# razvanmatisan/duodiff

Hardware: AMD Instinct MI355X
Metric: images/sec (whole node) DuoDiff 1000-step CelebA-64 (higher is better)
Workload: dtype bf16

## Files before the change

duodiff_amd/csrc/attention.hip:

```cpp
#include "dd_internal.h"

#include <type_traits>
#include <utility>

namespace dd {
namespace {

constexpr int kMaxKeyTiles = 9;
constexpr int kLP = kMaxKeyTiles * 32;
constexpr int kHD = 64;
constexpr int kPartBytes = 4 * 2 * 66 * 4;

__device__ __forceinline__ unsigned pack2_bf16(float lo, float hi) {
    typedef __bf16 bf16v2 __attribute__((ext_vector_type(2)));
    typedef float f32v2 __attribute__((ext_vector_type(2)));
    const f32v2 q = {lo, hi};
    return __builtin_bit_cast(unsigned, __builtin_convertvector(q, bf16v2));
}

__device__ __forceinline__ unsigned lds_addr_of(const void* p) {
    return (unsigned)(size_t)(const __attribute__((address_space(3))) char*)p;
}

__device__ __forceinline__ int k_swz(int r) { return ((r >> 1) & 7) ^ ((r & 1) << 2); }
__device__ __forceinline__ int v_swz(int r) { return (2 * (r & 3)) ^ ((r >> 2) & 1); }

template <typename T> struct AttnLayout;
template <> struct AttnLayout<bf16_t> {
    static constexpr int kRowK = 128;
    static constexpr int kRowV = 128;
    static constexpr int kVBytes = kLP * kRowV;
};
template <> struct AttnLayout<float> {
    static constexpr int kRowK = 256 + 16;
    static constexpr int kRowV = kLP * 4 + 16;
    static constexpr int kVBytes = kHD * kRowV;
};

template <typename T, int NKT, int NT, bool KPERM, typename TileFn>
__device__ __forceinline__ void attend_tiles(const char* Ks, const char* Vt, int L, int nkt, int lane, TileFn&& tile,
                                         const f32x4 (&qcur)[sizeof(T) == 2 ? 4 : 8], f32x16 (&o)[2], float& mx, float& sum) {
    using Lay = AttnLayout<T>;
    const int half = lane >> 5, r32 = lane & 31;
    const f32x16 zero16 = {0.f, 0.f, 0.f, 0.f, 0.f, 0.f, 0.f, 0.f, 0.f, 0.f, 0.f, 0.f, 0.f, 0.f, 0.f, 0.f};
    f32x16 s[NT];

    if constexpr (sizeof(T) == 2) {
        bf16x8 qf[4];
#pragma unroll
        for (int st = 0; st < 4; ++st) qf[st] = __builtin_bit_cast(bf16x8, qcur[st]);
        auto load_k = [&](int t, bf16x8 (&kf)[4]) {
            const char* kr = Ks + (t * 32 + r32) * Lay::kRowK;
            const int sw = k_swz(r32);
#pragma unroll
            for (int st = 0; st < 4; ++st) {
                const int ch = KPERM ? 4 * (st >> 1) + 2 * half + (st & 1) : 2 * st + half;
                kf[st] = *reinterpret_cast<const bf16x8*>(kr + ((ch ^ sw) << 4));
            }
        };
        bf16x8 kfa[4], kfb[4];
        if (tile(0) >= 0) load_k(tile(0), kfa);
#pragma unroll
        for (int k = 0; k < NT; ++k) {
            const int t = tile(k);
            const int tn = k + 1 < NT ? tile(k + 1) : -1;
            if (tn >= 0) { if (k & 1) load_k(tn, kfa); else load_k(tn, kfb); }
            __builtin_amdgcn_sched_barrier(0);
            if (t >= 0) {
                s[k] = __builtin_amdgcn_mfma_f32_32x32x16_bf16((k & 1) ? kfb[0] : kfa[0], qf[0], zero16, 0, 0, 0);
#pragma unroll
                for (int st = 1; st < 4; ++st)
                    s[k] = __builtin_amdgcn_mfma_f32_32x32x16_bf16((k & 1) ? kfb[st] : kfa[st], qf[st], s[k], 0, 0, 0);
            } else {
                s[k] = zero16;
            }
            __builtin_amdgcn_sched_barrier(0);
        }
    } else {
#pragma unroll
        for (int k = 0; k < NT; ++k) {
            const int t = tile(k);
            s[k] = zero16;
            if (t >= 0) {
                const char* kr = Ks + (t * 32 + r32) * Lay::kRowK + (32 * half) * 4;
#pragma unroll
                for (int g = 0; g < 8; ++g) {
                    const f32x4 kf = *reinterpret_cast<const f32x4*>(kr + g * 16);
#pragma unroll
                    for (int e = 0; e < 4; ++e)
                        s[k] = __builtin_amdgcn_mfma_f32_32x32x2f32(kf[e], qcur[g][e], s[k], 0, 0, 0);
                }
            }
        }
    }

    mx = -INFINITY;
#pragma unroll
    for (int k = 0; k < NT; ++k) {
        const int t = tile(k);
        if (t >= 0) {
            if (t == nkt - 1) {
#pragma unroll
                for (int e = 0; e < 16; ++e) {
                    const int key = t * 32 + (e & 3) + 8 * (e >> 2) + 4 * half;
                    if (key >= L) s[k][e] = -INFINITY;
                }
            }
#pragma unroll
            for (int e = 0; e < 16; ++e) mx = fmaxf(mx, s[k][e]);
        }
    }
    mx = fmaxf(mx, __shfl_xor(mx, 32));
    constexpr float kScaleLog2e = 0.125f * 1.4426950408889634f;
    const float mxs = mx * kScaleLog2e;
    sum = 0.f;
#pragma unroll
    for (int k = 0; k < NT; ++k) {
        if (tile(k) >= 0) {
#pragma unroll
            for (int e = 0; e < 16; ++e) {
                float p;
                if (NKT == 9 && NT == 9 && k == 8 && e >= 2) {
                    s[k][e] = 0.f;
                    continue;
                }
                if constexpr (sizeof(T) == 2) p = __builtin_amdgcn_exp2f(fmaf(s[k][e], kScaleLog2e, -mxs));
                else p = expf((s[k][e] - mx) * 0.125f);
                s[k][e] = p;
                sum += p;
            }
        }
    }
    sum += __shfl_xor(sum, 32);

    o[0] = zero16;
    o[1] = zero16;

    if constexpr (sizeof(T) == 2) {
        typedef __attribute__((ext_vector_type(4))) short s4;
        struct VF { s4 lo[2][2], hi[2][2]; };
        const int tq = (lane >> 2) & 3, tp = lane & 3, dhalf = (lane >> 4) & 1;
        const char* vb0 = Vt + (4 * half + tq) * Lay::kRowV + 8 * (tp & 1);
        const int vsw = v_swz(4 * half + tq);
        const char* vbd[2] = {vb0 + (((2 * dhalf + (tp >> 1)) ^ vsw) << 4), vb0 + (((4 + 2 * dhalf + (tp >> 1)) ^ vsw) << 4)};
        typedef __attribute__((address_space(3))) s4* lds_s4_ptr;
        auto load_v = [&](int t, VF& f) {
#pragma unroll
            for (int st = 0; st < 2; ++st)
#pragma unroll
                for (int dt = 0; dt < 2; ++dt) {
                    const char* vr = vbd[dt] + (t * 32 + 16 * st) * Lay::kRowV;
                    f.lo[st][dt] = __builtin_amdgcn_ds_read_tr16_b64_v4i16((lds_s4_ptr)(size_t)lds_addr_of(vr));
                    f.hi[st][dt] = __builtin_amdgcn_ds_read_tr16_b64_v4i16((lds_s4_ptr)(size_t)lds_addr_of(vr + 8 * Lay::kRowV));
                }
        };
        VF va, vb;
        if (tile(0) >= 0) load_v(tile(0), va);
#pragma unroll
        for (int k = 0; k < NT; ++k) {
            const int t = tile(k);
            const int tn = k + 1 < NT ? tile(k + 1) : -1;
            if (tn >= 0) { if (k & 1) load_v(tn, va); else load_v(tn, vb); }
            __builtin_amdgcn_sched_barrier(0);
            if (t >= 0) {
                const VF& f = (k & 1) ? vb : va;
#pragma unroll
                for (int st = 0; st < 2; ++st) {
                    bf16x8 pf;
#pragma unroll
                    for (int j = 0; j < 8; ++j) pf[j] = (short)f2bf(s[k][8 * st + j]);
#pragma unroll
                    for (int dt = 0; dt < 2; ++dt) {
                        bf16x8 vf;
#pragma unroll
                        for (int j = 0; j < 4; ++j) { vf[j] = f.lo[st][dt][j]; vf[4 + j] = f.hi[st][dt][j]; }
                        o[dt] = __builtin_amdgcn_mfma_f32_32x32x16_bf16(vf, pf, o[dt], 0, 0, 0);
                    }
                }
            }
            __builtin_amdgcn_sched_barrier(0);
        }
    } else {
#pragma unroll
        for (int k = 0; k < NT; ++k) {
            const int t = tile(k);
            if (t >= 0) {
#pragma unroll
                for (int g = 0; g < 4; ++g) {
#pragma unroll
                    for (int dt = 0; dt < 2; ++dt) {
                        const char* vr = Vt + (dt * 32 + r32) * Lay::kRowV + (t * 32 + 8 * g + 4 * half) * 4;
                        const f32x4 vf = *reinterpret_cast<const f32x4*>(vr);
#pragma unroll
                        for (int e = 0; e < 4; ++e)
                            o[dt] = __builtin_amdgcn_mfma_f32_32x32x2f32(vf[e], s[k][4 * g + e], o[dt], 0, 0, 0);
                    }
                }
            }
        }
    }
}

template <typename T, int NKT>
__global__ void __launch_bounds__(256, sizeof(T) == 2 ? 2 : 1)
attention_kernel(const T* __restrict__ qkv, T* __restrict__ out, int B, int L, int H, int D, int Lp) {
    using Lay = AttnLayout<T>;
    extern __shared__ __attribute__((aligned(16))) char smem[];
    char* Ks = smem;
    char* Vt = smem + kLP * Lay::kRowK;

    const int b = blockIdx.x / H, hh = blockIdx.x % H;
    const int tid = threadIdx.x, lane = tid & 63, wave = tid >> 6;
    const int half = lane >> 5, r32 = lane & 31;
    constexpr long long ld = kHD;
    const long long unit = (long long)Lp * kHD;
    const T* qbase = qkv + ((long long)b * 3 * H + hh) * unit;
    const T* kbase = qbase + (long long)H * unit;
    const T* vbase = kbase + (long long)H * unit;
    const int nkt = NKT > 0 ? NKT : (L + 31) / 32;
    constexpr int EPC = 16 / (int)sizeof(T);
    constexpr int CPR = kHD / EPC;

    constexpr int NQF = sizeof(T) == 2 ? 4 : 8;
    auto load_q = [&](int qc, f32x4 (&qf)[NQF]) {
        const int q = qc * 32 + r32;
        const T* qrow = qbase + (long long)(q < L ? q : L - 1) * ld;
#pragma unroll
        for (int i = 0; i < NQF; ++i)
            qf[i] = sizeof(T) == 2 ? *reinterpret_cast<const f32x4*>(qrow + 16 * i + 8 * half)
                                   : *reinterpret_cast<const f32x4*>(qrow + 32 * half + 4 * i);
    };
    f32x4 qnext[NQF];
    load_q(wave, qnext);

    if constexpr (sizeof(T) == 2) {
        typedef const __attribute__((address_space(1))) void* gptr_t;
        typedef __attribute__((address_space(3))) void* lptr_t;
        const int np = Lp >> 3;
        const int wv = __builtin_amdgcn_readfirstlane(wave);
        const int lr = lane >> 3, slot = lane & 7;
        constexpr int MAXP = (kLP / 8 * 2 + 3) / 4;
#pragma unroll
        for (int i = 0; i < MAXP; ++i) {
            const int p2 = wv + 4 * i;
            if (p2 < 2 * np) {
                const bool isv = p2 >= np;
                const int p = isv ? p2 - np : p2, r = 8 * p + lr;
                const int ch = isv ? (slot ^ v_swz(r)) : (slot ^ k_swz(r));
                const T* src = (isv ? vbase : kbase) + (long long)(r < L ? r : L - 1) * kHD + ch * 8;
                char* dst = (isv ? Vt : Ks) + p * 1024;
                __builtin_amdgcn_global_load_lds((gptr_t)src, (lptr_t)dst, 16, 0, 0);
            }
        }
        for (int i = tid; i < (nkt * 32 - Lp) * 16; i += 256) {
            const int rr = Lp + (i >> 4), c = i & 15;
            *reinterpret_cast<f32x4*>((c < 8 ? Ks : Vt) + rr * 128 + (c & 7) * 16) = f32x4{0.f, 0.f, 0.f, 0.f};
        }
        asm volatile("s_waitcnt vmcnt(0)" ::: "memory");
    } else {
        for (int idx = tid; idx < nkt * 32 * CPR; idx += 256) {
            const int key = idx / CPR, ch = idx % CPR;
            f32x4 kv = {0.f, 0.f, 0.f, 0.f}, vv = {0.f, 0.f, 0.f, 0.f};
            if (key < L) {
                kv = *reinterpret_cast<const f32x4*>(kbase + (long long)key * ld + ch * EPC);
                vv = *reinterpret_cast<const f32x4*>(vbase + (long long)key * ld + ch * EPC);
            }
            *reinterpret_cast<f32x4*>(Ks + key * Lay::kRowK + ch * 16) = kv;
            T tmp[EPC];
            *reinterpret_cast<f32x4*>(tmp) = vv;
#pragma unroll
            for (int e = 0; e < EPC; ++e)
                *reinterpret_cast<T*>(Vt + (ch * EPC + e) * Lay::kRowV + key * (int)sizeof(T)) = tmp[e];
        }
    }

    __syncthreads();

    constexpr bool SPLIT_LAST = NKT == 9;
    const int nqc = (L + 31) / 32;
    const int n_regular = SPLIT_LAST ? 8 : nqc;
    for (int qc = wave; qc < n_regular; qc += 4) {
        const int q = qc * 32 + r32;
        f32x4 qcur[NQF];
#pragma unroll
        for (int i = 0; i < NQF; ++i) qcur[i] = qnext[i];
        if (qc + 4 < n_regular) load_q(qc + 4, qnext);
        else if (SPLIT_LAST) load_q(8, qnext);

        f32x16 o[2];
        float mx, sum;
        attend_tiles<T, NKT, kMaxKeyTiles, false>(Ks, Vt, L, nkt, lane, [&](int k) { return k < nkt ? k : -1; }, qcur, o, mx, sum);
        const float inv = 1.0f / sum;

        T* orow = out + ((long long)b * L + (q < L ? q : L - 1)) * D + hh * kHD;
        if constexpr (sizeof(T) == 2) {
#pragma unroll
            for (int dt = 0; dt < 2; ++dt) {
                uint2 v[4];
#pragma unroll
                for (int g = 0; g < 4; ++g) {
                    bf16_t v4[4];
#pragma unroll
                    for (int e = 0; e < 4; ++e) v4[e] = f2bf(o[dt][4 * g + e] * inv);
                    v[g] = *reinterpret_cast<const uint2*>(v4);
                }
#pragma unroll
                for (int gp = 0; gp < 4; gp += 2) {
                    const auto s0 = __builtin_amdgcn_permlane32_swap(v[gp].x, v[gp + 1].x, false, false);
                    const auto s1 = __builtin_amdgcn_permlane32_swap(v[gp].y, v[gp + 1].y, false, false);
                    const uint4 o4 = {s0[0], s1[0], s0[1], s1[1]};
                    if (q < L) *reinterpret_cast<uint4*>(orow + dt * 32 + 8 * gp + 8 * half) = o4;
                }
            }
        } else if (q < L) {
#pragma unroll
            for (int dt = 0; dt < 2; ++dt)
#pragma unroll
                for (int g = 0; g < 4; ++g) {
                    const int d = dt * 32 + 8 * g + 4 * half;
                    *reinterpret_cast<f32x4*>(orow + d) = f32x4{o[dt][4 * g] * inv, o[dt][4 * g + 1] * inv, o[dt][4 * g + 2] * inv, o[dt][4 * g + 3] * inv};
                }
        }
    }

    if constexpr (SPLIT_LAST) {
        float* part = reinterpret_cast<float*>(smem + kLP * Lay::kRowK + Lay::kVBytes);
        const int rem = L - 256;
        f32x16 o[2];
        float mx, sum;
        attend_tiles<T, NKT, 3, false>(Ks, Vt, L, nkt, lane, [&](int k) { return k < 2 ? wave + 4 * k : (wave == 3 ? 8 : -1); }, qnext, o, mx, sum);
        if (r32 < rem) {
            float* pw = part + (wave * 2 + r32) * 66;
#pragma unroll
            for (int dt = 0; dt < 2; ++dt)
#pragma unroll
                for (int g = 0; g < 4; ++g)
                    *reinterpret_cast<f32x4*>(pw + dt * 32 + 8 * g + 4 * half) =
                        f32x4{o[dt][4 * g], o[dt][4 * g + 1], o[dt][4 * g + 2], o[dt][4 * g + 3]};
            if (half == 0) { pw[64] = mx; pw[65] = sum; }
        }
        __syncthreads();
        if (tid < rem * 64) {
            const int qi = tid >> 6, d = tid & 63;
            float m[4], M = -INFINITY;
#pragma unroll
            for (int w = 0; w < 4; ++w) { m[w] = part[(w * 2 + qi) * 66 + 64]; M = fmaxf(M, m[w]); }
            float num = 0.f, den = 0.f;
#pragma unroll
            for (int w = 0; w < 4; ++w) {
                float f;
                if constexpr (sizeof(T) == 2) f = __builtin_amdgcn_exp2f((m[w] - M) * (0.125f * 1.4426950408889634f));
                else f = expf((m[w] - M) * 0.125f);
                num = fmaf(f, part[(w * 2 + qi) * 66 + d], num);
                den = fmaf(f, part[(w * 2 + qi) * 66 + 65], den);
            }
            out[((long long)b * L + 256 + qi) * D + hh * kHD + d] = Elem<T>::from_f32(num / den);
        }
    }
}


struct QkvAttnArgs {
    const bf16_t* h;
    const bf16_t* wimg;
    const float* bias;
    const bf16_t* hx;
    const float* xres;
    const float* ln_g;
    const float* ln_b;
    bf16_t* out;
    int B, L, H, Lp, E;
};

constexpr int kQaPxBytes = 8 * 6 * 2 * 32 * 4;
constexpr int kQaHxPad = 64;
constexpr int kQaHxBytes = 2 * (1024 * 2 + kQaHxPad);
constexpr int kQaAuxBytes = kQaPxBytes + kQaHxBytes + 256;
constexpr int kQaKQ = 8;
constexpr int kQaBlk = 2 * kQaKQ * 1024;
constexpr int kQaRing = 4 * kQaBlk;
static_assert(8 * 2 * 66 * 4 <= kQaPxBytes, "the split chunk's partials reuse the px area");

typedef const __attribute__((address_space(1))) void* qa_gptr_t;
typedef __attribute__((address_space(3))) void* qa_lptr_t;

constexpr int qa_dma_ops(int b, int nb) { return b < nb ? 2 : 0; }
constexpr int qa_pref_ops(int b, int nb) { return (b >= 0 && b % 3 == 0 && b / 3 + 1 < nb / 3) ? kQaKQ : 0; }
constexpr int qa_younger_dma(int b, int nb) { return qa_pref_ops(b - 1, nb) + qa_dma_ops(b + 2, nb) + qa_pref_ops(b, nb); }
constexpr int qa_younger_rows(int b, int nb) { return qa_dma_ops(b, nb) + qa_dma_ops(b + 1, nb) + qa_dma_ops(b + 2, nb); }

template <int D>
__global__ void __launch_bounds__(512, 1) qkv_attention_kernel(const QkvAttnArgs a) {
    using Lay = AttnLayout<bf16_t>;
    constexpr int KS = D / 16, NS = KS / kQaKQ, NB = 3 * NS;
    static_assert(D % 128 == 0 && D >= 512 && D <= 1024, "k range in slices of 8 k-steps; hxl holds two rows of D <= 1024");
    extern __shared__ __attribute__((aligned(16))) char smem[];
    char* Ks = smem;
    char* Vt = smem + kLP * Lay::kRowK;
    float* px = reinterpret_cast<float*>(smem + kLP * Lay::kRowK + Lay::kVBytes);
    float* part = px;
    char* hxl = smem + kLP * Lay::kRowK + Lay::kVBytes + kQaPxBytes;
    char* qxl = hxl + kQaHxBytes;
    char* ring = smem + kLP * Lay::kRowK + Lay::kVBytes + kQaAuxBytes;

    int b, hh;
    if ((a.B & 7) == 0) { const int slot = blockIdx.x >> 3; b = (blockIdx.x & 7) + 8 * (slot / a.H); hh = slot % a.H; }
    else { b = blockIdx.x / a.H; hh = blockIdx.x % a.H; }
    const int tid = threadIdx.x, lane = tid & 63, wave = __builtin_amdgcn_readfirstlane(tid >> 6);
    const int half = lane >> 5, r32 = lane & 31;
    const int L = a.L, E = a.E;

    const char* wsrc = reinterpret_cast<const char*>(a.wimg) + (size_t)hh * NB * kQaBlk;
    const unsigned lane16 = lane * 16;
    auto dma_block = [&](int bb) {
#pragma unroll
        for (int i = 0; i < 2; ++i) {
            const int pc = wave * 2 + i;
            const char* sb = wsrc + (size_t)bb * kQaBlk + pc * 1024;
            const unsigned lds = lds_addr_of(ring + (bb & 3) * kQaBlk + pc * 1024);
            asm volatile("s_mov_b32 m0, %0\n\tglobal_load_lds_dwordx4 %1, %2" ::"s"(lds), "v"(lane16), "s"(sb) : "memory", "m0");
        }
    };
    dma_block(0);
    dma_block(1);
    dma_block(2);

    const int row = 32 * wave + r32;
    const bf16x8* hfr_u = reinterpret_cast<const bf16x8*>(a.h) + ((long long)b * 8 + wave) * KS * 64;
    const bf16x8* hfr = hfr_u + lane;
    bf16x8 xs[2][kQaKQ];
#pragma unroll
    for (int ks = 0; ks < kQaKQ; ++ks) xs[0][ks] = hfr[ks * 64];

    if (a.hx) {
        for (int i = tid; i < E * (D / 8); i += 512) {
            const int e = i / (D / 8), cch = i % (D / 8);
            *reinterpret_cast<f32x4*>(hxl + e * (D * 2 + kQaHxPad) + cch * 16) = *reinterpret_cast<const f32x4*>(a.hx + ((long long)b * L + e) * D + cch * 8);
        }
    } else if (wave < E) {
        constexpr int NV = D / 256;
        const float* xr = a.xres + ((long long)b * L + wave) * D + lane * (D / 64);
        f32x4 xv[NV];
        float s1 = 0.f;
#pragma unroll
        for (int v = 0; v < NV; ++v) {
            xv[v] = *reinterpret_cast<const f32x4*>(xr + 4 * v);
            s1 += (xv[v][0] + xv[v][1]) + (xv[v][2] + xv[v][3]);
        }
#pragma unroll
        for (int o = 32; o >= 1; o >>= 1) s1 += __shfl_xor(s1, o);
        const float mean = s1 / (float)D;
        float s2 = 0.f;
#pragma unroll
        for (int v = 0; v < NV; ++v) {
            xv[v] = xv[v] - mean;
            s2 += (xv[v][0] * xv[v][0] + xv[v][1] * xv[v][1]) + (xv[v][2] * xv[v][2] + xv[v][3] * xv[v][3]);
        }
#pragma unroll
        for (int o = 32; o >= 1; o >>= 1) s2 += __shfl_xor(s2, o);
        const float rstd = 1.0f / sqrtf(s2 / (float)D + 1e-5f);
#pragma unroll
        for (int v = 0; v < NV; ++v) {
            const f32x4 g = *reinterpret_cast<const f32x4*>(a.ln_g + lane * (D / 64) + 4 * v), c0 = *reinterpret_cast<const f32x4*>(a.ln_b + lane * (D / 64) + 4 * v);
            const f32x4 y = xv[v] * rstd * g + c0;
            *reinterpret_cast<uint2*>(hxl + wave * (D * 2 + kQaHxPad) + (lane * (D / 64) + 4 * v) * 2) = uint2{pack2_bf16(y[0], y[1]), pack2_bf16(y[2], y[3])};
        }
    }
    for (int i = tid; i < (kLP - 256 - E) * 16; i += 512) {
        const int r = 256 + E + (i >> 4), c = i & 15;
        *reinterpret_cast<f32x4*>((c < 8 ? Ks : Vt) + r * 128 + (c & 7) * 16) = f32x4{0.f, 0.f, 0.f, 0.f};
    }

    const f32x16 zero16 = {0.f, 0.f, 0.f, 0.f, 0.f, 0.f, 0.f, 0.f, 0.f, 0.f, 0.f, 0.f, 0.f, 0.f, 0.f, 0.f};
    f32x16 acc[6];
#pragma unroll
    for (int j = 0; j < 6; ++j) acc[j] = zero16;
    f32x4 accx[6];
#pragma unroll
    for (int j = 0; j < 6; ++j) accx[j] = f32x4{0.f, 0.f, 0.f, 0.f};
    const int xg = lane >> 4, xn = lane & 15;
    const int wx16 = (2 * (wave >> 1) + (xg >> 1)) * 1024 + ((16 * (wave & 1) + xn) + 32 * (xg & 1)) * 16;
    const char* hx16 = hxl + (xn < E ? xn : 0) * (D * 2 + kQaHxPad) + (wave >> 1) * 64 + xg * 16;
    bf16x8 wq[4];
    asm volatile("s_waitcnt vmcnt(0)\n\ts_waitcnt lgkmcnt(0)\n\ts_barrier" ::: "memory");
#pragma unroll
    for (int i = 0; i < 4; ++i) wq[i] = *reinterpret_cast<const bf16x8*>(ring + lane * 16 + i * 1024);
    [&]<int... BI>(std::integer_sequence<int, BI...>) {
        ([&] {
            constexpr int bb = BI, q = bb / 3, jj = bb % 3, S = q & 1;
            if constexpr (jj == 0) {
                if constexpr (q > 0) {
                    asm volatile("s_waitcnt vmcnt(%8)"
                                 : "+v"(xs[S][0]), "+v"(xs[S][1]), "+v"(xs[S][2]), "+v"(xs[S][3]), "+v"(xs[S][4]), "+v"(xs[S][5]), "+v"(xs[S][6]), "+v"(xs[S][7])
                                 : "i"(qa_younger_rows(bb, NB)));
                }
                if constexpr (q + 1 < NS) {
#pragma unroll
                    for (int ks = 0; ks < kQaKQ; ++ks)
                        asm volatile("global_load_dwordx4 %0, %1, %2" : "=v"(xs[S ^ 1][ks]) : "v"(lane16), "s"(hfr_u + ((q + 1) * kQaKQ + ks) * 64) : "memory");
                }
            }
            const char* wb = ring + (bb & 3) * kQaBlk + lane * 16;
            const char* wbn = ring + ((bb + 1) & 3) * kQaBlk + lane * 16;
#pragma unroll
            for (int f = 0; f < 2 * kQaKQ; ++f) {
                if (f == kQaKQ) {
                    if constexpr (bb + 1 < NB) {
                        if constexpr (bb + 1 >= 3) asm volatile("s_waitcnt vmcnt(%0)\n\ts_barrier" ::"i"(qa_younger_dma(bb, NB)) : "memory");
                        else asm volatile("s_barrier" ::: "memory");
                    }
                    if constexpr (bb + 3 < NB) dma_block(bb + 3);
                    const bf16x8 hb = *reinterpret_cast<const bf16x8*>(hx16 + q * (kQaKQ * 32));
#pragma unroll
                    for (int t = 0; t < 2; ++t) {
                        const bf16x8 wa = *reinterpret_cast<const bf16x8*>(ring + (bb & 3) * kQaBlk + t * (kQaKQ * 1024) + wx16);
                        accx[2 * jj + t] = __builtin_amdgcn_mfma_f32_16x16x32_bf16(wa, hb, accx[2 * jj + t], 0, 0, 0);
                    }
                }
                const bf16x8 w0 = wq[f & 3];
                if (f + 4 < 2 * kQaKQ) wq[f & 3] = *reinterpret_cast<const bf16x8*>(wb + (f + 4) * 1024);
                else if (bb + 1 < NB) wq[f & 3] = *reinterpret_cast<const bf16x8*>(wbn + (f + 4 - 2 * kQaKQ) * 1024);
                acc[2 * jj + (f >> 3)] = __builtin_amdgcn_mfma_f32_32x32x16_bf16(w0, xs[S][f & 7], acc[2 * jj + (f >> 3)], 0, 0, 0);
            }
        }(), ...);
    }(std::make_integer_sequence<int, NB>{});

    if (xn < E) {
#pragma unroll
        for (int j = 0; j < 6; ++j) *reinterpret_cast<f32x4*>(px + (((wave * 6 + j) * 2 + xn) * 16 + 4 * xg)) = accx[j];
    }
    f32x4 qcur[4];
    const int swk = k_swz(row), swv = v_swz(row);
#pragma unroll
    for (int j = 0; j < 6; ++j) {
        if (a.bias) {
            const float* bj = a.bias + (j >> 1) * D + hh * kHD + 32 * (j & 1) + 4 * half;
#pragma unroll
            for (int g = 0; g < 4; ++g) {
                const f32x4 bv = *reinterpret_cast<const f32x4*>(bj + 8 * g);
#pragma unroll
                for (int e = 0; e < 4; ++e) acc[j][4 * g + e] += bv[e];
            }
        }
        unsigned pk[8];
#pragma unroll
        for (int i = 0; i < 8; ++i) pk[i] = pack2_bf16(acc[j][2 * i], acc[j][2 * i + 1]);
        const int T = j & 1;
        if (j < 2) {
            qcur[2 * T] = __builtin_bit_cast(f32x4, uint4{pk[0], pk[1], pk[2], pk[3]});
            qcur[2 * T + 1] = __builtin_bit_cast(f32x4, uint4{pk[4], pk[5], pk[6], pk[7]});
        } else if (j < 4) {
            *reinterpret_cast<uint4*>(Ks + row * 128 + (((4 * T + 2 * half) ^ swk) << 4)) = uint4{pk[0], pk[1], pk[2], pk[3]};
            *reinterpret_cast<uint4*>(Ks + row * 128 + (((4 * T + 2 * half + 1) ^ swk) << 4)) = uint4{pk[4], pk[5], pk[6], pk[7]};
        } else {
#pragma unroll
            for (int gp = 0; gp < 4; gp += 2) {
                const auto s0 = __builtin_amdgcn_permlane32_swap(pk[2 * gp], pk[2 * gp + 2], false, false);
                const auto s1 = __builtin_amdgcn_permlane32_swap(pk[2 * gp + 1], pk[2 * gp + 3], false, false);
                *reinterpret_cast<uint4*>(Vt + row * 128 + (((4 * T + gp + half) ^ swv) << 4)) = uint4{s0[0], s1[0], s0[1], s1[1]};
            }
        }
    }
    __syncthreads();
    if (tid < E * 192) {
        const int e = tid / 192, c = tid % 192, j = c >> 5, col = c & 31;
        float v = a.bias ? a.bias[(j >> 1) * D + hh * kHD + 32 * (j & 1) + col] : 0.f;
#pragma unroll
        for (int kb = 0; kb < 4; ++kb) v += px[(((2 * kb + (col >> 4)) * 6 + j) * 2 + e) * 16 + (col & 15)];
        const bf16_t vb = f2bf(v);
        const int d = 32 * (j & 1) + col, r = 256 + e;
        if (j < 2) {
            *reinterpret_cast<bf16_t*>(qxl + e * 128 + d * 2) = vb;
        } else if (j < 4) {
            const int T = d >> 5, dd = d & 31, hf = (dd >> 2) & 1, ae = (dd & 3) + 4 * (dd >> 3);
            *reinterpret_cast<bf16_t*>(Ks + r * 128 + (((4 * T + 2 * hf + (ae >> 3)) ^ k_swz(r)) << 4) + (ae & 7) * 2) = vb;
        } else {
            *reinterpret_cast<bf16_t*>(Vt + r * 128 + (((d >> 3) ^ v_swz(r)) << 4) + (d & 7) * 2) = vb;
        }
    }
    __syncthreads();

    f32x4 qe[4];
    {
        const bf16_t* qrow = reinterpret_cast<const bf16_t*>(qxl) + (r32 < E ? r32 : E - 1) * kHD + 4 * half;
#pragma unroll
        for (int st = 0; st < 4; ++st) {
            const uint2 lo = *reinterpret_cast<const uint2*>(qrow + 32 * (st >> 1) + 16 * (st & 1));
            const uint2 hi = *reinterpret_cast<const uint2*>(qrow + 32 * (st >> 1) + 16 * (st & 1) + 8);
            qe[st] = __builtin_bit_cast(f32x4, uint4{lo.x, lo.y, hi.x, hi.y});
        }
    }

    {
        f32x16 o[2];
        float mx, sum;
        attend_tiles<bf16_t, 9, kMaxKeyTiles, true>(Ks, Vt, L, kMaxKeyTiles, lane, [&](int k) { return k; }, qcur, o, mx, sum);
        const float inv = 1.0f / sum;
        bf16_t* orow = a.out + ((long long)b * L + E + row) * D + hh * kHD;
#pragma unroll
        for (int dt = 0; dt < 2; ++dt) {
            uint2 v[4];
#pragma unroll
            for (int g = 0; g < 4; ++g) {
                bf16_t v4[4];
#pragma unroll
                for (int e = 0; e < 4; ++e) v4[e] = f2bf(o[dt][4 * g + e] * inv);
                v[g] = *reinterpret_cast<const uint2*>(v4);
            }
#pragma unroll
            for (int gp = 0; gp < 4; gp += 2) {
                const auto s0 = __builtin_amdgcn_permlane32_swap(v[gp].x, v[gp + 1].x, false, false);
                const auto s1 = __builtin_amdgcn_permlane32_swap(v[gp].y, v[gp + 1].y, false, false);
                *reinterpret_cast<uint4*>(orow + dt * 32 + 8 * gp + 8 * half) = uint4{s0[0], s1[0], s0[1], s1[1]};
            }
        }
    }

    {
        f32x16 o[2];
        float mx, sum;
        attend_tiles<bf16_t, 9, 2, true>(Ks, Vt, L, kMaxKeyTiles, lane, [&](int k) { return k == 0 ? wave : (wave == 7 ? 8 : -1); }, qe, o, mx, sum);
        if (r32 < E) {
            float* pw = part + (wave * 2 + r32) * 66;
#pragma unroll
            for (int dt = 0; dt < 2; ++dt)
#pragma unroll
                for (int g = 0; g < 4; ++g)
                    *reinterpret_cast<f32x4*>(pw + dt * 32 + 8 * g + 4 * half) =
                        f32x4{o[dt][4 * g], o[dt][4 * g + 1], o[dt][4 * g + 2], o[dt][4 * g + 3]};
            if (half == 0) { pw[64] = mx; pw[65] = sum; }
        }
        __syncthreads();
        if (tid < E * 64) {
            const int qi = tid >> 6, d = tid & 63;
            float m[8], M = -INFINITY;
#pragma unroll
            for (int w = 0; w < 8; ++w) { m[w] = part[(w * 2 + qi) * 66 + 64]; M = fmaxf(M, m[w]); }
            float num = 0.f, den = 0.f;
#pragma unroll
            for (int w = 0; w < 8; ++w) {
                const float f = __builtin_amdgcn_exp2f((m[w] - M) * (0.125f * 1.4426950408889634f));
                num = fmaf(f, part[(w * 2 + qi) * 66 + d], num);
                den = fmaf(f, part[(w * 2 + qi) * 66 + 65], den);
            }
            a.out[((long long)b * L + qi) * D + hh * kHD + d] = f2bf(num / den);
        }
    }
}

}

template <typename T>
hipError_t launch_attention(const T* qkv, T* out, int B, int L, int H, int D, hipStream_t s) {
    if (L > kLP || D != H * kHD || L < 1) return hipErrorInvalidValue;
    using Lay = AttnLayout<T>;
    const size_t lds = (size_t)kLP * Lay::kRowK + (size_t)Lay::kVBytes + kPartBytes;
    const int Lp = make_head_major(L, H).Lp;
    if (L == 257 || L == 258) hipLaunchKernelGGL((attention_kernel<T, 9>), dim3(B * H), dim3(256), lds, s, qkv, out, B, L, H, D, Lp);
    else hipLaunchKernelGGL((attention_kernel<T, 0>), dim3(B * H), dim3(256), lds, s, qkv, out, B, L, H, D, Lp);
    return hipGetLastError();
}

void qkv_attention_pack(int D, int H, const float* w, unsigned short (*to_bf16)(float), unsigned short* img) {
    const int NS = D / 16 / kQaKQ;
    for (int hh = 0; hh < H; ++hh)
        for (int q = 0; q < NS; ++q)
            for (int j = 0; j < 6; ++j)
                for (int ks = 0; ks < kQaKQ; ++ks)
                    for (int lane = 0; lane < 64; ++lane) {
                        const float* src = w + ((size_t)(j >> 1) * D + 64 * hh + 32 * (j & 1) + (lane & 31)) * D + 16 * (q * kQaKQ + ks) + 8 * (lane >> 5);
                        unsigned short* dst = img + (((((size_t)hh * NS + q) * 6 + j) * kQaKQ + ks) * 64 + lane) * 8;
                        for (int i = 0; i < 8; ++i) dst[i] = to_bf16(src[i]);
                    }
}

bool qkv_attention_supported(int D, int H, int L, int extras) {
    return (D == 512 || D == 768 || D == 1024) && H * kHD == D && (extras == 1 || extras == 2) && L == 256 + extras;
}

static size_t qkv_attention_lds() { return (size_t)kLP * AttnLayout<bf16_t>::kRowK + AttnLayout<bf16_t>::kVBytes + kQaAuxBytes + kQaRing; }

hipError_t launch_qkv_attention(const bf16_t* h, const bf16_t* wimg, const float* bias, const bf16_t* hx, const float* xres,
                                const float* ln_g, const float* ln_b, bf16_t* out, int B, int L, int H, int D, int extras, hipStream_t s) {
    if (!qkv_attention_supported(D, H, L, extras) || !h || !wimg || (!hx && (!xres || !ln_g || !ln_b)) || !out || B < 1) return hipErrorInvalidValue;
    const QkvAttnArgs a{h, wimg, bias, hx, xres, ln_g, ln_b, out, B, L, H, make_head_major(L, H).Lp, extras};
    switch (D) {
        case 512: hipLaunchKernelGGL((qkv_attention_kernel<512>), dim3(B * H), dim3(512), qkv_attention_lds(), s, a); break;
        case 768: hipLaunchKernelGGL((qkv_attention_kernel<768>), dim3(B * H), dim3(512), qkv_attention_lds(), s, a); break;
        default: hipLaunchKernelGGL((qkv_attention_kernel<1024>), dim3(B * H), dim3(512), qkv_attention_lds(), s, a); break;
    }
    return hipGetLastError();
}

hipError_t init_attention_kernels() {
    for (const void* f : {(const void*)qkv_attention_kernel<512>, (const void*)qkv_attention_kernel<768>, (const void*)qkv_attention_kernel<1024>})
        if (hipError_t e = hipFuncSetAttribute(f, hipFuncAttributeMaxDynamicSharedMemorySize, (int)qkv_attention_lds()); e != hipSuccess) return e;
    const int lb = kLP * AttnLayout<bf16_t>::kRowK + AttnLayout<bf16_t>::kVBytes + kPartBytes;
    const int lf = kLP * AttnLayout<float>::kRowK + AttnLayout<float>::kVBytes + kPartBytes;
    hipError_t e = hipFuncSetAttribute((const void*)attention_kernel<bf16_t, 9>, hipFuncAttributeMaxDynamicSharedMemorySize, lb);
    if (e == hipSuccess) e = hipFuncSetAttribute((const void*)attention_kernel<bf16_t, 0>, hipFuncAttributeMaxDynamicSharedMemorySize, lb);
    if (e == hipSuccess) e = hipFuncSetAttribute((const void*)attention_kernel<float, 9>, hipFuncAttributeMaxDynamicSharedMemorySize, lf);
    if (e == hipSuccess) e = hipFuncSetAttribute((const void*)attention_kernel<float, 0>, hipFuncAttributeMaxDynamicSharedMemorySize, lf);
    return e;
}

template hipError_t launch_attention<bf16_t>(const bf16_t*, bf16_t*, int, int, int, int, hipStream_t);
template hipError_t launch_attention<float>(const float*, float*, int, int, int, int, hipStream_t);

}
```

duodiff_amd/csrc/gemm.hip:

```cpp
#include "dd_internal.h"

#include <type_traits>

namespace dd {

namespace {

typedef const __attribute__((address_space(1))) void* gptr_t;
typedef __attribute__((address_space(3))) void* lptr_t;

__device__ __forceinline__ void glds16(const void* src, void* lds_dst) {
    __builtin_amdgcn_global_load_lds((gptr_t)src, (lptr_t)lds_dst, 16, 0, 0);
}

__device__ __forceinline__ float gelu_erf_f32(float v) { return 0.5f * v * (1.0f + erff(v * 0.70710678118654752440f)); }

__device__ __forceinline__ void glds16s(const char* sbase, unsigned voff, const void* lds_dst) {
    const unsigned lds = (unsigned)(size_t)(const __attribute__((address_space(3))) char*)lds_dst;
    asm volatile("s_mov_b32 m0, %0\n\tglobal_load_lds_dwordx4 %1, %2" ::"s"(lds), "v"(voff), "s"(sbase) : "memory", "m0");
}

template <int ROWS, int NWAVES>
__device__ __forceinline__ void stage_tile(const char* g, long long row_stride, char* lds_tile,
                                           int wave, int lane, int row_limit) {
    constexpr int PER_WAVE = ROWS / 8 / NWAVES;
#pragma unroll
    for (int j = 0; j < PER_WAVE; ++j) {
        const int inst = wave * PER_WAVE + j;
        int r = inst * 8 + (lane >> 3);
        const int c = (lane & 7) ^ ((r >> 1) & 7);
        r = r < row_limit ? r : row_limit - 1;
        glds16(g + (long long)r * row_stride + c * 16, lds_tile + inst * 1024);
    }
}

template <typename T>
__device__ __forceinline__ f32x4 gelu_erf4(f32x4 v) {
    if constexpr (sizeof(T) == 4) {
        f32x4 r;
#pragma unroll
        for (int e = 0; e < 4; ++e) r[e] = gelu_erf_f32(v[e]);
        return r;
    } else {
        f32x4 sc;
#pragma unroll
        for (int i = 0; i < 4; ++i) sc[i] = __builtin_amdgcn_fmed3f(v[i], -3.8f, 3.8f);
        const f32x4 s2 = sc * sc;
        f32x4 p = s2 * 7.331517960e-08f + -4.544908101e-06f;
        p = p * s2 + 1.213693460e-04f;
        p = p * s2 + -1.863093246e-03f;
        p = p * s2 + 1.863326334e-02f;
        p = p * s2 + -1.314395642e-01f;
        p = p * s2 + 7.973534865e-01f;
        const f32x4 e = p * sc;
        const f32x4 hv = v * 0.5f;
        return hv * e + hv;
    }
}

__device__ __forceinline__ f32x4 lds_read16(const char* p) {
    return *reinterpret_cast<const f32x4*>(p);
}

template <typename T>
__device__ __forceinline__ void mma_chunk(f32x16& acc, const f32x4& a, const f32x4& b);

template <>
__device__ __forceinline__ void mma_chunk<bf16_t>(f32x16& acc, const f32x4& a, const f32x4& b) {
    acc = __builtin_amdgcn_mfma_f32_32x32x16_bf16(__builtin_bit_cast(bf16x8, a),
                                                  __builtin_bit_cast(bf16x8, b), acc, 0, 0, 0);
}
template <>
__device__ __forceinline__ void mma_chunk<float>(f32x16& acc, const f32x4& a, const f32x4& b) {
#pragma unroll
    for (int e = 0; e < 4; ++e) acc = __builtin_amdgcn_mfma_f32_32x32x2f32(a[e], b[e], acc, 0, 0, 0);
}

template <int N>
__device__ __forceinline__ void wait_vmcnt() {
    asm volatile("s_waitcnt vmcnt(%0)" ::"i"(N) : "memory");
}

template <typename T, int BM, int BN, int WM, int WN, int STAGES, int EPI>
__global__ void __launch_bounds__(WM* WN * 64)
gemm_kernel(const GemmArgs<T> a) {
    constexpr int NW = WM * WN;
    constexpr int TM = BM / WM / 32, TN = BN / WN / 32;
    constexpr int KT_ELEMS = 128 / (int)sizeof(T);
    constexpr int A_BYTES = BM * 128, B_BYTES = BN * 128;
    constexpr int STAGE_BYTES = A_BYTES + B_BYTES;
    constexpr int G = (BM + BN) / 8 / NW;
    extern __shared__ __attribute__((aligned(16))) char smem[];

    const int lane = threadIdx.x & 63;
    const int wave = __builtin_amdgcn_readfirstlane(threadIdx.x >> 6);
    const int wr = wave / WN, wc = wave % WN;
    const int h = lane >> 5, r32 = lane & 31;

    const int n_tiles = (a.N + BN - 1) / BN;
    int wg = blockIdx.x;
    {
        const int nwg = gridDim.x, xcd = wg & 7, q = nwg >> 3, r = nwg & 7;
        wg = (xcd < r ? xcd * (q + 1) : r * (q + 1) + (xcd - r) * q) + (wg >> 3);
    }
    const int tile_m = wg / n_tiles, tile_n = wg % n_tiles;
    const int m0 = tile_m * BM, n0 = tile_n * BN;
    const int n_limit = a.N - n0;
    const int m_limit = a.M - m0 < BM ? a.M - m0 : BM;

    const int nk = a.K / KT_ELEMS;
    const int nk1 = a.K1 / KT_ELEMS;
    const char* A1 = reinterpret_cast<const char*>(a.A) + (long long)m0 * a.lda * sizeof(T);
    const char* A2 = a.A2 ? reinterpret_cast<const char*>(a.A2) + (long long)m0 * a.lda2 * sizeof(T) : nullptr;
    const char* Wp = reinterpret_cast<const char*>(a.W) + (long long)n0 * a.K * sizeof(T);
    const long long sa1 = (long long)a.lda * sizeof(T), sa2 = (long long)a.lda2 * sizeof(T);
    const long long sw = (long long)a.K * sizeof(T);

    auto stage = [&](int kt, int buf) {
        char* at = smem + buf * STAGE_BYTES;
        if (kt < nk1) stage_tile<BM, NW>(A1 + (long long)kt * 128, sa1, at, wave, lane, m_limit);
        else stage_tile<BM, NW>(A2 + (long long)(kt - nk1) * 128, sa2, at, wave, lane, m_limit);
        stage_tile<BN, NW>(Wp + (long long)kt * 128, sw, at + A_BYTES, wave, lane, n_limit);
    };

    f32x16 acc[TM][TN];
#pragma unroll
    for (int i = 0; i < TM; ++i)
#pragma unroll
        for (int j = 0; j < TN; ++j)
#pragma unroll
            for (int e = 0; e < 16; ++e) acc[i][j][e] = 0.f;

    auto compute = [&](int buf) {
        const char* Ab = smem + buf * STAGE_BYTES + (wr * (BM / WM)) * 128;
        const char* Bb = smem + buf * STAGE_BYTES + A_BYTES + (wc * (BN / WN)) * 128;
#pragma unroll
        for (int step = 0; step < 4; ++step) {
            const int chunk = sizeof(T) == 2 ? (2 * step + h) : (4 * h + step);
            f32x4 af[TM], bfr[TN];
#pragma unroll
            for (int i = 0; i < TM; ++i) {
                const int r = i * 32 + r32;
                const int tr = wr * (BM / WM) + r;
                af[i] = lds_read16(Ab + r * 128 + ((chunk ^ ((tr >> 1) & 7)) << 4));
            }
#pragma unroll
            for (int j = 0; j < TN; ++j) {
                const int r = j * 32 + r32;
                const int tr = wc * (BN / WN) + r;
                bfr[j] = lds_read16(Bb + r * 128 + ((chunk ^ ((tr >> 1) & 7)) << 4));
            }
#pragma unroll
            for (int i = 0; i < TM; ++i)
#pragma unroll
                for (int j = 0; j < TN; ++j) mma_chunk<T>(acc[i][j], bfr[j], af[i]);
        }
    };

    if constexpr (STAGES == 2) {
        stage(0, 0);
        __syncthreads();
        for (int kt = 0; kt < nk; ++kt) {
            const int cur = kt & 1;
            if (kt + 1 < nk) stage(kt + 1, cur ^ 1);
            compute(cur);
            __syncthreads();
        }
    } else {
#pragma unroll
        for (int s = 0; s < STAGES - 1; ++s)
            if (s < nk) stage(s, s);
        int rd = 0, wrb = STAGES - 1;
// ... 511 lines not shown
```

duodiff_amd/csrc/rowlin.hip:

```cpp
#include "dd_internal.h"

#include <utility>

namespace dd {
namespace {

typedef const __attribute__((address_space(1))) void* rl_gptr_t;
typedef __attribute__((address_space(3))) void* rl_lptr_t;

constexpr int kRlD = 768, kRlNT = kRlD / 32, kRlBlk = kRlNT * 1024;
constexpr int kRlRing = 4 * kRlBlk;
constexpr int kRlABuf = 128 * 128;
constexpr int kRlLds = kRlRing + 3 * kRlABuf;

__device__ __forceinline__ unsigned rl_pack2(float lo, float hi) {
    typedef __bf16 bf16v2 __attribute__((ext_vector_type(2)));
    typedef float f32v2 __attribute__((ext_vector_type(2)));
    const f32v2 q = {lo, hi};
    return __builtin_bit_cast(unsigned, __builtin_convertvector(q, bf16v2));
}

__device__ __forceinline__ unsigned rl_lds(const void* p) { return (unsigned)(size_t)(const __attribute__((address_space(3))) char*)p; }
__device__ __forceinline__ void rl_dma(const char* sbase, unsigned voff, const void* lds_dst) {
    asm volatile("s_mov_b32 m0, %0\n\tglobal_load_lds_dwordx4 %1, %2" ::"s"(rl_lds(lds_dst)), "v"(voff), "s"(sbase) : "memory", "m0");
}
template <int OFF>
__device__ __forceinline__ void rl_read(bf16x8& d, unsigned addr) {
    asm volatile("ds_read_b128 %0, %1 offset:%2" : "=v"(d) : "v"(addr), "i"(OFF));
}
template <int LG, int LO, bool AGPR>
__device__ __forceinline__ void rl_gap(f32x16& acc, bf16x8& wa, const bf16x8& xb, unsigned la) {
    if constexpr (AGPR)
        asm volatile("s_waitcnt lgkmcnt(%4)\n\tv_mfma_f32_32x32x16_bf16 %0, %1, %2, %0\n\tds_read_b128 %1, %3 offset:%5"
                     : "+a"(acc), "+v"(wa) : "v"(xb), "v"(la), "i"(LG), "i"(LO));
    else
        asm volatile("s_waitcnt lgkmcnt(%4)\n\tv_mfma_f32_32x32x16_bf16 %0, %1, %2, %0\n\tds_read_b128 %1, %3 offset:%5"
                     : "+v"(acc), "+v"(wa) : "v"(xb), "v"(la), "i"(LG), "i"(LO));
}
constexpr int kRlNA = 16;
template <int T>
__device__ __forceinline__ void rl_pin(f32x16& y) {
    if constexpr (T < kRlNA) asm volatile("" : "+a"(y));
    else asm volatile("" : "+v"(y));
}

__global__ void __launch_bounds__(256) rowlin768_kernel(const RowLinArgs a) {
    extern __shared__ __attribute__((aligned(16))) char smem[];
    char* ring = smem;
    char* abuf = smem + kRlRing;
    const int tid = threadIdx.x, lane = tid & 63, wave = __builtin_amdgcn_readfirstlane(tid >> 6);
    const int h = lane >> 5, r32 = lane & 31;
    const bool planned = a.tok_n > 0;
    const bool part_tile = planned && (int)blockIdx.x >= a.tiles_main;
    const int xe = part_tile ? (int)blockIdx.x - a.tiles_main : 0;
    const int tile = part_tile ? xe / a.groups : (int)blockIdx.x;
    const int ks0 = part_tile ? (xe % a.groups) * a.cpg : 0;
    const int ks_all = a.K >> 4;
    const int KS = part_tile ? (ks0 + a.cpg < ks_all ? a.cpg : ks_all - ks0) : ks_all, NG = KS >> 2;
    auto row_of = [&](int local, bool& ok) -> long long {
        const int idx = tile * 128 + local;
        if (!planned) { ok = idx < a.M; return ok ? idx : a.M - 1; }
        if (!part_tile) {
            ok = idx < a.n_main;
            const int p = ok ? idx : a.n_main - 1, b = p / a.tok_n;
            return (long long)b * a.tok_l + a.tok_e + (p - b * a.tok_n);
        }
        ok = idx < a.n_extra;
        const int q = ok ? idx : a.n_extra - 1, b = q / a.tok_e;
        return (long long)b * a.tok_l + (q - b * a.tok_e);
    };

    const char* wsrc = a.wimg + (size_t)ks0 * kRlBlk;
    const unsigned lane16 = lane * 16;
    auto dma_w = [&](int ks) {
#pragma unroll
        for (int i = 0; i < 6; ++i) {
            const int pc = wave * 6 + i;
            rl_dma(wsrc + (size_t)ks * kRlBlk + pc * 1024, lane16, ring + (ks & 3) * kRlBlk + pc * 1024);
        }
    };
    const int lr = lane >> 3;
    unsigned arows[4];
    const char* abase_1 = reinterpret_cast<const char*>(a.A);
    const char* abase_2 = a.k_split > 0 ? reinterpret_cast<const char*>(a.A2) - (long long)a.k_split * 2 : abase_1;
    const int g_split = a.k_split > 0 ? (a.k_split >> 6) - (ks0 >> 2) : (1 << 30);
#pragma unroll
    for (int i = 0; i < 4; ++i) {
        bool okr;
        const int r = (wave * 4 + i) * 8 + lr;
        arows[i] = (unsigned)((row_of(r, okr) * a.lda + (long long)ks0 * 16) * 2) + (((lane & 7) ^ ((r >> 1) & 7)) << 4);
    }
    auto dma_a = [&](int g) {
#pragma unroll
        for (int i = 0; i < 4; ++i) {
            const int pc = wave * 4 + i;
            rl_dma(g < g_split ? abase_1 : abase_2, arows[i] + (unsigned)g * 128u, abuf + (g % 3) * kRlABuf + pc * 1024);
        }
    };
    auto dma_w1 = [&](int ks, int j) {
        const int pc = wave * 6 + j;
        rl_dma(wsrc + (size_t)ks * kRlBlk + pc * 1024, lane16, ring + (ks & 3) * kRlBlk + pc * 1024);
    };
    auto dma_a1 = [&](int g, int j) {
        const int pc = wave * 4 + j;
        rl_dma(g < g_split ? abase_1 : abase_2, arows[j] + (unsigned)g * 128u, abuf + (g % 3) * kRlABuf + pc * 1024);
    };
    dma_a(0);
    dma_a(1);
    dma_w(0);
    dma_w(1);
    dma_w(2);

    f32x16 Y[kRlNT];
    const f32x16 zero16 = {0.f, 0.f, 0.f, 0.f, 0.f, 0.f, 0.f, 0.f, 0.f, 0.f, 0.f, 0.f, 0.f, 0.f, 0.f, 0.f};
    [&]<int... T>(std::integer_sequence<int, T...>) { ((Y[T] = zero16, rl_pin<T>(Y[T])), ...); }(std::make_integer_sequence<int, kRlNT>{});

    const int arow = 32 * wave + r32;
    const unsigned afr = rl_lds(abuf) + arow * 128;
    const int asw = (arow >> 1) & 7;
    const unsigned wlo = rl_lds(ring) + lane * 16, whi = wlo + 65536u;

    asm volatile("s_waitcnt vmcnt(0)\n\ts_barrier" ::: "memory");
    constexpr int PD = 8;
    bf16x8 wa[PD], xf[2];
    rl_read<0>(xf[0], afr + ((h ^ asw) << 4));
    [&]<int... J>(std::integer_sequence<int, J...>) { (rl_read<J * 1024>(wa[J], wlo), ...); }(std::make_integer_sequence<int, PD>{});
    for (int g = 0; g < NG; ++g) {
        const bool more_a = g + 2 < NG;
        const unsigned abase = afr + (unsigned)(g % 3) * kRlABuf, anext = afr + (unsigned)((g + 1) % 3) * kRlABuf;
        [&]<int... GI>(std::integer_sequence<int, GI...>) {
            ([&] {
                constexpr int gi = GI, i = gi / kRlNT, t = gi % kRlNT;
                const int ks = 4 * g + i;
                if constexpr (t == 2) {
                    if (ks + 2 >= KS) asm volatile("s_waitcnt vmcnt(0)\n\ts_barrier" ::: "memory");
                    else if (i == 1 && more_a) asm volatile("s_waitcnt vmcnt(10)\n\ts_barrier" ::: "memory");
                    else if (i == 2 && more_a) asm volatile("s_waitcnt vmcnt(7)\n\ts_barrier" ::: "memory");
                    else asm volatile("s_waitcnt vmcnt(6)\n\ts_barrier" ::: "memory");
                }
                if constexpr (t >= 3 && t <= 18 && t % 3 == 0) { if (ks + 3 < KS) dma_w1(ks + 3, (t - 3) / 3); }
                if constexpr (i == 0 && (t == 4 || t == 10 || t == 16 || t == 22)) { if (more_a) dma_a1(g + 2, (t - 4) / 6); }
                if constexpr (t == kRlNT / 2) {
                    const unsigned na = (i < 3 ? abase : anext) + ((((2 * ((i + 1) & 3)) + h) ^ asw) << 4);
                    rl_read<0>(xf[(i + 1) & 1], na);
                }
                constexpr int tn = t + PD, sl = tn < kRlNT ? i : ((i + 1) & 3), tt = tn < kRlNT ? tn : tn - kRlNT;
                constexpr int LO = sl * kRlBlk + tt * 1024;
                rl_gap<PD - 1, (LO < 65536 ? LO : LO - 65536), (t < kRlNA)>(Y[t], wa[gi % PD], xf[i & 1], LO < 65536 ? wlo : whi);
            }(), ...);
        }(std::make_integer_sequence<int, 4 * kRlNT>{});
    }
    asm volatile("s_waitcnt lgkmcnt(0)\n\ts_nop 15\n\ts_nop 15" ::: "memory");
    [&]<int... T>(std::integer_sequence<int, T...>) { (rl_pin<T>(Y[T]), ...); }(std::make_integer_sequence<int, kRlNT>{});

    asm volatile("s_barrier" ::: "memory");
    constexpr int kPitch = 1024 + 16;
    char* strip = smem + wave * (32 * kPitch);
    bool ok;
    const long long rr = row_of(arow, ok);
    bool ok0;
    const long long row0w = __builtin_amdgcn_readfirstlane((int)row_of(32 * wave, ok0));
    const int limit = !planned ? a.M : a.n_main;
    const long long rows_all = planned ? (long long)(a.n_main / a.tok_n) * a.tok_l : a.M;
    int nvalid = limit - (tile * 128 + 32 * wave);
    nvalid = part_tile ? 32 : (nvalid < 0 ? 0 : (nvalid > 32 ? 32 : nvalid));
    const float keep = part_tile || a.set_x ? 0.f : 1.f, keepb = part_tile ? 0.f : 1.f;
    ok = ok || part_tile;
    f32x4 s4 = {0.f, 0.f, 0.f, 0.f}, q4 = {0.f, 0.f, 0.f, 0.f};
    float cshift = 0.f;
#pragma unroll
    for (int p = 0; p < 3; ++p) {
        if (a.set_x || part_tile) {
#pragma unroll
            for (int j = 0; j < 32; ++j) *reinterpret_cast<f32x4*>(strip + r32 * kPitch + (h * 32 + j) * 16) = f32x4{0.f, 0.f, 0.f, 0.f};
        } else {
            const char* src = reinterpret_cast<const char*>(a.xres + 256 * p);
            for (int i = 0; i < nvalid; ++i) {
// ... 130 lines not shown
```

Measured before the change: 48.77.

## Split attention into score/softmax/PV phases and interleave main and extra-token paths

Splits the attention helper into separate score, softmax and PV stages. The fused kernel now runs the main-query and extra-query attention phase by phase, so their independent MFMA and LDS work can interleave. This is meant to hide latency in the tail kernel, at the cost of more live registers. It also inserts an s_nop between the m0 write and global_load_lds in every DMA helper, likely a hazard or correctness fix that adds one cycle per issue.

Result: no change. 48.81 (median of 6 runs) (+0.1%).

```diff
diff --git a/duodiff_amd/csrc/attention.hip b/duodiff_amd/csrc/attention.hip
--- a/duodiff_amd/csrc/attention.hip
+++ b/duodiff_amd/csrc/attention.hip
@@ -37,13 +37,11 @@
     static constexpr int kVBytes = kHD * kRowV;
 };
 
-template <typename T, int NKT, int NT, bool KPERM, typename TileFn>
-__device__ __forceinline__ void attend_tiles(const char* Ks, const char* Vt, int L, int nkt, int lane, TileFn&& tile,
-                                         const f32x4 (&qcur)[sizeof(T) == 2 ? 4 : 8], f32x16 (&o)[2], float& mx, float& sum) {
+template <typename T, int NT, bool KPERM, typename TileFn>
+__device__ __forceinline__ void score_tiles(const char* Ks, int lane, TileFn&& tile, const f32x4 (&qcur)[sizeof(T) == 2 ? 4 : 8], f32x16 (&s)[NT]) {
     using Lay = AttnLayout<T>;
     const int half = lane >> 5, r32 = lane & 31;
     const f32x16 zero16 = {0.f, 0.f, 0.f, 0.f, 0.f, 0.f, 0.f, 0.f, 0.f, 0.f, 0.f, 0.f, 0.f, 0.f, 0.f, 0.f};
-    f32x16 s[NT];
 
     if constexpr (sizeof(T) == 2) {
         bf16x8 qf[4];
@@ -93,7 +91,11 @@
             }
         }
     }
-
+}
+
+template <typename T, int NKT, int NT, typename TileFn>
+__device__ __forceinline__ void softmax_tiles(int L, int nkt, int lane, TileFn&& tile, f32x16 (&s)[NT], float& mx, float& sum) {
+    const int half = lane >> 5;
     mx = -INFINITY;
 #pragma unroll
     for (int k = 0; k < NT; ++k) {
@@ -132,7 +134,13 @@
         }
     }
     sum += __shfl_xor(sum, 32);
-
+}
+
+template <typename T, int NT, typename TileFn>
+__device__ __forceinline__ void pv_tiles(const char* Vt, int lane, TileFn&& tile, const f32x16 (&s)[NT], f32x16 (&o)[2]) {
+    using Lay = AttnLayout<T>;
+    const int half = lane >> 5, r32 = lane & 31;
+    const f32x16 zero16 = {0.f, 0.f, 0.f, 0.f, 0.f, 0.f, 0.f, 0.f, 0.f, 0.f, 0.f, 0.f, 0.f, 0.f, 0.f, 0.f};
     o[0] = zero16;
     o[1] = zero16;
 
@@ -199,6 +207,15 @@
             }
         }
     }
+}
+
+template <typename T, int NKT, int NT, bool KPERM, typename TileFn>
+__device__ __forceinline__ void attend_tiles(const char* Ks, const char* Vt, int L, int nkt, int lane, TileFn&& tile,
+                                         const f32x4 (&qcur)[sizeof(T) == 2 ? 4 : 8], f32x16 (&o)[2], float& mx, float& sum) {
+    f32x16 s[NT];
+    score_tiles<T, NT, KPERM>(Ks, lane, tile, qcur, s);
+    softmax_tiles<T, NKT, NT>(L, nkt, lane, tile, s, mx, sum);
+    pv_tiles<T, NT>(Vt, lane, tile, s, o);
 }
 
 template <typename T, int NKT>
@@ -418,7 +435,7 @@
             const int pc = wave * 2 + i;
             const char* sb = wsrc + (size_t)bb * kQaBlk + pc * 1024;
             const unsigned lds = lds_addr_of(ring + (bb & 3) * kQaBlk + pc * 1024);
-            asm volatile("s_mov_b32 m0, %0\n\tglobal_load_lds_dwordx4 %1, %2" ::"s"(lds), "v"(lane16), "s"(sb) : "memory", "m0");
+            asm volatile("s_mov_b32 m0, %0\n\ts_nop 0\n\tglobal_load_lds_dwordx4 %1, %2" ::"s"(lds), "v"(lane16), "s"(sb) : "memory", "m0");
         }
     };
     dma_block(0);
@@ -580,21 +597,28 @@
     }
     __syncthreads();
 
-    f32x4 qe[4];
     {
-        const bf16_t* qrow = reinterpret_cast<const bf16_t*>(qxl) + (r32 < E ? r32 : E - 1) * kHD + 4 * half;
-#pragma unroll
-        for (int st = 0; st < 4; ++st) {
-            const uint2 lo = *reinterpret_cast<const uint2*>(qrow + 32 * (st >> 1) + 16 * (st & 1));
-            const uint2 hi = *reinterpret_cast<const uint2*>(qrow + 32 * (st >> 1) + 16 * (st & 1) + 8);
-            qe[st] = __builtin_bit_cast(f32x4, uint4{lo.x, lo.y, hi.x, hi.y});
-        }
-    }
-
-    {
-        f32x16 o[2];
-        float mx, sum;
-        attend_tiles<bf16_t, 9, kMaxKeyTiles, true>(Ks, Vt, L, kMaxKeyTiles, lane, [&](int k) { return k; }, qcur, o, mx, sum);
+        auto all_tiles = [&](int k) { return k; };
+        auto x_tiles = [&](int k) { return k == 0 ? wave : (wave == 7 ? 8 : -1); };
+        f32x16 s[kMaxKeyTiles], se[2];
+        score_tiles<bf16_t, kMaxKeyTiles, true>(Ks, lane, all_tiles, qcur, s);
+        f32x4 qe[4];
+        {
+            const bf16_t* qrow = reinterpret_cast<const bf16_t*>(qxl) + (r32 < E ? r32 : E - 1) * kHD + 4 * half;
+#pragma unroll
+            for (int st = 0; st < 4; ++st) {
+                const uint2 lo = *reinterpret_cast<const uint2*>(qrow + 32 * (st >> 1) + 16 * (st & 1));
+                const uint2 hi = *reinterpret_cast<const uint2*>(qrow + 32 * (st >> 1) + 16 * (st & 1) + 8);
+                qe[st] = __builtin_bit_cast(f32x4, uint4{lo.x, lo.y, hi.x, hi.y});
+            }
+        }
+        score_tiles<bf16_t, 2, true>(Ks, lane, x_tiles, qe, se);
+        float mx, sum, mxe, sume;
+        softmax_tiles<bf16_t, 9, kMaxKeyTiles>(L, kMaxKeyTiles, lane, all_tiles, s, mx, sum);
+        softmax_tiles<bf16_t, 9, 2>(L, kMaxKeyTiles, lane, x_tiles, se, mxe, sume);
+        f32x16 o[2], oe[2];
+        pv_tiles<bf16_t, kMaxKeyTiles>(Vt, lane, all_tiles, s, o);
+        pv_tiles<bf16_t, 2>(Vt, lane, x_tiles, se, oe);
         const float inv = 1.0f / sum;
         bf16_t* orow = a.out + ((long long)b * L + E + row) * D + hh * kHD;
 #pragma unroll
@@ -614,12 +638,6 @@
                 *reinterpret_cast<uint4*>(orow + dt * 32 + 8 * gp + 8 * half) = uint4{s0[0], s1[0], s0[1], s1[1]};
             }
         }
-    }
-
-    {
-        f32x16 o[2];
-        float mx, sum;
-        attend_tiles<bf16_t, 9, 2, true>(Ks, Vt, L, kMaxKeyTiles, lane, [&](int k) { return k == 0 ? wave : (wave == 7 ? 8 : -1); }, qe, o, mx, sum);
         if (r32 < E) {
             float* pw = part + (wave * 2 + r32) * 66;
 #pragma unroll
@@ -627,24 +645,25 @@
 #pragma unroll
                 for (int g = 0; g < 4; ++g)
                     *reinterpret_cast<f32x4*>(pw + dt * 32 + 8 * g + 4 * half) =
-                        f32x4{o[dt][4 * g], o[dt][4 * g + 1], o[dt][4 * g + 2], o[dt][4 * g + 3]};
-            if (half == 0) { pw[64] = mx; pw[65] = sum; }
-        }
-        __syncthreads();
-        if (tid < E * 64) {
-            const int qi = tid >> 6, d = tid & 63;
-            float m[8], M = -INFINITY;
-#pragma unroll
-            for (int w = 0; w < 8; ++w) { m[w] = part[(w * 2 + qi) * 66 + 64]; M = fmaxf(M, m[w]); }
-            float num = 0.f, den = 0.f;
-#pragma unroll
-            for (int w = 0; w < 8; ++w) {
-                const float f = __builtin_amdgcn_exp2f((m[w] - M) * (0.125f * 1.4426950408889634f));
-                num = fmaf(f, part[(w * 2 + qi) * 66 + d], num);
-                den = fmaf(f, part[(w * 2 + qi) * 66 + 65], den);
-            }
-            a.out[((long long)b * L + qi) * D + hh * kHD + d] = f2bf(num / den);
-        }
+                        f32x4{oe[dt][4 * g], oe[dt][4 * g + 1], oe[dt][4 * g + 2], oe[dt][4 * g + 3]};
+            if (half == 0) { pw[64] = mxe; pw[65] = sume; }
+        }
+    }
+
+    __syncthreads();
+    if (tid < E * 64) {
+        const int qi = tid >> 6, d = tid & 63;
+        float m[8], M = -INFINITY;
+#pragma unroll
+        for (int w = 0; w < 8; ++w) { m[w] = part[(w * 2 + qi) * 66 + 64]; M = fmaxf(M, m[w]); }
+        float num = 0.f, den = 0.f;
+#pragma unroll
+        for (int w = 0; w < 8; ++w) {
+            const float f = __builtin_amdgcn_exp2f((m[w] - M) * (0.125f * 1.4426950408889634f));
+            num = fmaf(f, part[(w * 2 + qi) * 66 + d], num);
+            den = fmaf(f, part[(w * 2 + qi) * 66 + 65], den);
+        }
+        a.out[((long long)b * L + qi) * D + hh * kHD + d] = f2bf(num / den);
     }
 }
 
diff --git a/duodiff_amd/csrc/gemm.hip b/duodiff_amd/csrc/gemm.hip
--- a/duodiff_amd/csrc/gemm.hip
+++ b/duodiff_amd/csrc/gemm.hip
@@ -17,7 +17,7 @@
 
 __device__ __forceinline__ void glds16s(const char* sbase, unsigned voff, const void* lds_dst) {
     const unsigned lds = (unsigned)(size_t)(const __attribute__((address_space(3))) char*)lds_dst;
-    asm volatile("s_mov_b32 m0, %0\n\tglobal_load_lds_dwordx4 %1, %2" ::"s"(lds), "v"(voff), "s"(sbase) : "memory", "m0");
+    asm volatile("s_mov_b32 m0, %0\n\ts_nop 0\n\tglobal_load_lds_dwordx4 %1, %2" ::"s"(lds), "v"(voff), "s"(sbase) : "memory", "m0");
 }
 
 template <int ROWS, int NWAVES>
diff --git a/duodiff_amd/csrc/rowlin.hip b/duodiff_amd/csrc/rowlin.hip
--- a/duodiff_amd/csrc/rowlin.hip
+++ b/duodiff_amd/csrc/rowlin.hip
@@ -22,7 +22,7 @@
 
 __device__ __forceinline__ unsigned rl_lds(const void* p) { return (unsigned)(size_t)(const __attribute__((address_space(3))) char*)p; }
 __device__ __forceinline__ void rl_dma(const char* sbase, unsigned voff, const void* lds_dst) {
-    asm volatile("s_mov_b32 m0, %0\n\tglobal_load_lds_dwordx4 %1, %2" ::"s"(rl_lds(lds_dst)), "v"(voff), "s"(sbase) : "memory", "m0");
+    asm volatile("s_mov_b32 m0, %0\n\ts_nop 0\n\tglobal_load_lds_dwordx4 %1, %2" ::"s"(rl_lds(lds_dst)), "v"(voff), "s"(sbase) : "memory", "m0");
 }
 template <int OFF>
 __device__ __forceinline__ void rl_read(bf16x8& d, unsigned addr) {
```
